# craftsangjae/instance-segmentation-road-project

Hardware: AMD Instinct MI355X
Metric: images/sec at 1024x1024 (MaskLab inference hot path, full forward) (higher is better)
Workload: dtype f32

## Files before the change

include/masklab_hip.h:

```cpp
#ifndef MASKLAB_HIP_H
#define MASKLAB_HIP_H

#include <stdint.h>

#ifdef __cplusplus
extern "C" {
#endif

#define ML_OK 0
#define ML_E_BADARG (-1)
#define ML_E_LAUNCH (-2)
#define ML_E_NOGPU  (-3)

enum { ML_ACT_NONE = 0, ML_ACT_RELU = 1, ML_ACT_RELU6 = 2, ML_ACT_SIGMOID = 3 };
enum { ML_MATH_F32 = 0, ML_MATH_F16 = 1, ML_MATH_F16S = 2, ML_MATH_F32X3 = 3 };

#define ML_ABI_VERSION 7
int ml_version(void);
const char *ml_last_error(void);
int ml_device_check(void);

typedef struct ml_conv2d_desc {
    const float *in;
    const float *wgt;
    const float *bias;
    const float *residual;
    float *out;
    int32_t B, H, W;
    int32_t in_cstride, in_coff;
    int32_t span;
    int32_t span_pad;
    int32_t cpp_shift;
    int32_t Ho, Wo;
    int32_t KH, KW, stride, dil, pad_t, pad_l;
    int32_t cout;
    int32_t n_pad;
    int32_t out_cstride, out_coff;
    int32_t res_cstride, res_coff;
    int32_t act;
    int32_t group_cin_step;
    int32_t shuffle2x2;
    int32_t tile;
    int32_t math;
    int32_t out_f16;
    int64_t out_bstride;
    const int32_t *live;
    int32_t live_period;
    int32_t reserved1;
    double *gn_partials;
} ml_conv2d_desc;

int ml_conv2d_f32(const ml_conv2d_desc *d, void *stream);

#define ML_CONV_MAX_PROBLEMS 12
int64_t ml_conv2d_workspace_bytes(void);
int ml_conv2d_multi_f32(const ml_conv2d_desc *descs, int32_t n, void *workspace, int64_t workspace_bytes,
                        void *stream);
int ml_conv2d_ntile(int32_t cout, int32_t tile);
int ml_conv2d_launch_ntile(const ml_conv2d_desc *descs, int32_t n, int32_t has_workspace);
int ml_conv2d_launch_mtile(const ml_conv2d_desc *descs, int32_t n, int32_t has_workspace);
int ml_conv2d_uses_pipe(const ml_conv2d_desc *d);
int ml_conv2d_launch_splits(const ml_conv2d_desc *descs, int32_t n, int64_t workspace_bytes, int32_t *splits);
int ml_conv2d_wino_eligible(const ml_conv2d_desc *d);
int64_t ml_conv2d_gn_min_launch_tiles(void);

int ml_gconv3x3_f32(const float *in, const float *wgt, const float *bias, float *out,
                    int32_t B, int32_t H, int32_t W, int32_t C, int32_t c, int32_t Ho, int32_t Wo,
                    int32_t stride, int32_t pad_t, int32_t pad_l, int32_t act, void *stream);

int ml_gconv3x3_f16(const void *in, const float *wgt, const float *bias, void *out,
                    int32_t B, int32_t H, int32_t W, int32_t C, int32_t c, int32_t Ho, int32_t Wo,
                    int32_t stride, int32_t pad_t, int32_t pad_l, int32_t act, void *stream);

int ml_maxpool3x3s2_f16(const void *in, void *out, int32_t B, int32_t H, int32_t W, int32_t C,
                        int32_t Ho, int32_t Wo, int32_t pad_t, int32_t pad_l, void *stream);
int ml_subsample2_f16(const void *in, void *out, int32_t B, int32_t H, int32_t W, int32_t C, void *stream);
int ml_cast_f16_to_f32(const void *in, float *out, int64_t n, void *stream);
int ml_cast_f32_to_f16(const float *in, void *out, int64_t n, void *stream);
int ml_resize_bilinear_ac_f16(const void *in, const void *add, void *out,
                              int32_t B, int32_t H, int32_t W, int32_t C, int32_t in_cstride, int32_t in_coff,
                              int32_t Ho, int32_t Wo, int32_t add_cstride, int32_t add_coff,
                              int32_t out_cstride, int32_t out_coff, void *stream);
int ml_dwconv3x3_f16(const void *in, const float *wgt, const float *bias, void *out,
                     int32_t B, int32_t H, int32_t W, int32_t C, int32_t in_cstride, int32_t in_coff,
                     int32_t out_cstride, int32_t out_coff, int32_t Ho, int32_t Wo,
                     int32_t stride, int32_t dil, int32_t pad_t, int32_t pad_l, int32_t act, void *stream);
int ml_global_mean_f16(const void *in, void *out, int32_t B, int32_t HW, int32_t C, void *stream);

int ml_stem7x7s2_pool_f16(const float *image, const void *wgt_h, const float *bias, void *out, int32_t B, int32_t H,
                          int32_t W, int32_t Hp, int32_t Wp, void *stream);
int ml_stem7x7s2_pool_f32(const float *image, const float *wgt, const float *bias, float *out, int32_t B, int32_t H,
                          int32_t W, int32_t Hp, int32_t Wp, void *stream);
int ml_stem7x7s2_pool_x3(const float *image, const void *wgt_x3, const float *bias, float *out, int32_t B, int32_t H,
                         int32_t W, int32_t Hp, int32_t Wp, void *stream);

typedef struct ml_deconv_out_problem {
    const float *x, *wd, *bd, *wo_table, *bo;
    float *out;
    int64_t M;
    int32_t hw, w, rois_per_image, reserved0;
    int64_t out_image_stride, out_base;
    const int32_t *live;
} ml_deconv_out_problem;
int ml_deconv2x2_out1x1_f32(const ml_deconv_out_problem *probs, int32_t nprob, int32_t K, int32_t c_mid, int32_t ncls,
                            int32_t cp, int32_t act_mid, int32_t act_out, void *stream);
int ml_deconv2x2_out1x1_f16(const ml_deconv_out_problem *probs, int32_t nprob, int32_t K, int32_t c_mid, int32_t ncls,
                            int32_t cp, int32_t act_mid, int32_t act_out, void *stream);

int ml_dwconv3x3_f32(const float *in, const float *wgt, const float *bias, float *out,
                     int32_t B, int32_t H, int32_t W, int32_t C,
                     int32_t in_cstride, int32_t in_coff, int32_t out_cstride, int32_t out_coff,
                     int32_t Ho, int32_t Wo, int32_t stride, int32_t dil,
                     int32_t pad_t, int32_t pad_l, int32_t act, void *stream);

int ml_maxpool3x3s2_f32(const float *in, float *out, int32_t B, int32_t H, int32_t W, int32_t C,
                        int32_t Ho, int32_t Wo, int32_t pad_t, int32_t pad_l, void *stream);
// ... 259 lines not shown
```

instance-segmentation-road-project_amd/csrc/conv_wino.hip:

```cpp
#include "common.h"

namespace {

constexpr int WMAXP = ML_CONV_MAX_PROBLEMS;
constexpr int WT = 64;
constexpr int WN = 64;
constexpr int WK = 8;
constexpr int WCHUNK = WK * 32 * 16;
constexpr int WSTEP = 4 * 32 * 16;
constexpr int NSLOT_P = 3;
constexpr int SLOT_P = WT * 16 * 8;
constexpr int NSLOT_W = 4;
constexpr int SLOT_W = 2 * WSTEP;
constexpr int RING_W = NSLOT_P * SLOT_P;
constexpr int LDS_BYTES = (RING_W + NSLOT_W * SLOT_W) * 4;
static_assert(LDS_BYTES == 160 * 1024, "the two rings fill the CU's LDS");
#ifndef WINO_EXP
#define WINO_EXP 0
#endif
constexpr unsigned OOB = 0x80000000u;
constexpr long long SPAN_MAX = 0x7fffff00ll;

struct WProblem {
    ml_conv2d_desc d;
    int TH, TW, T;
    int MB, NB, nchunks;
};

struct WArgs {
    int n;
    int start[WMAXP + 1];
    WProblem p[WMAXP];
};

__device__ __forceinline__ void dma16(__amdgpu_buffer_rsrc_t rsrc, float *dst, int voff) {
#if defined(__HIP_DEVICE_COMPILE__)
    __builtin_amdgcn_raw_ptr_buffer_load_lds(rsrc, (__attribute__((address_space(3))) void *)dst, 16, voff, 0, 0, 0);
#endif
}

__device__ __forceinline__ void bt_d_b_op(int k, const float d[16], float t[16], float v[16]) {
    if (k < 16) {
        const int j = k >> 2;
        switch (k & 3) {
            case 0: t[0 * 4 + j] = d[0 * 4 + j] - d[2 * 4 + j]; break;
            case 1: t[1 * 4 + j] = d[1 * 4 + j] + d[2 * 4 + j]; break;
            case 2: t[2 * 4 + j] = d[2 * 4 + j] - d[1 * 4 + j]; break;
            default: t[3 * 4 + j] = d[1 * 4 + j] - d[3 * 4 + j]; break;
        }
    } else {
        const int i = (k - 16) >> 2;
        switch (k & 3) {
            case 0: v[i * 4 + 0] = t[i * 4 + 0] - t[i * 4 + 2]; break;
            case 1: v[i * 4 + 1] = t[i * 4 + 1] + t[i * 4 + 2]; break;
            case 2: v[i * 4 + 2] = t[i * 4 + 2] - t[i * 4 + 1]; break;
            default: v[i * 4 + 3] = t[i * 4 + 1] - t[i * 4 + 3]; break;
        }
    }
}

__global__ void __launch_bounds__(512, 1) conv_wino_kernel(const WArgs args) {
    extern __shared__ __align__(16) float lds[];

    int pi = 0;
    while (pi + 1 < args.n && (int)blockIdx.x >= args.start[pi + 1]) ++pi;
    const WProblem &P = args.p[pi];
    const ml_conv2d_desc &p = P.d;
    const int b = (int)blockIdx.x - args.start[pi];
    const int g = b / (8 * P.NB), rr = b - g * 8 * P.NB;
    const int nt2 = rr >> 3;
    const int mt = g * 8 + (rr & 7);
    if (mt >= P.MB) return;
    if (p.live) {
        const int lv = max(1, *p.live), tpi0 = P.TH * P.TW;
        const int b0 = mt * WT / tpi0, b1 = min(mt * WT + WT, P.T) - 1;
        bool any = false;
        for (int bi = b0; bi <= b1 / tpi0 && !any; ++bi) any = bi % p.live_period < lv;
        if (!any) return;
    }

    const int tid = threadIdx.x, lane = tid & 63;
    const int wave = __builtin_amdgcn_readfirstlane(tid >> 6);
    const int tg = wave & 3, h = wave >> 2;
    const int r = lane & 15, kq = lane >> 4;
    const int tpi = P.TH * P.TW;

    const int gt0 = mt * WT;
    long long base_pix;
    {
        const int bi = gt0 / tpi, rem = gt0 - bi * tpi, ty = rem / P.TW;
        base_pix = ((long long)bi * p.H + max(2 * ty - 1, 0)) * p.W;
    }
    const size_t cstride = (size_t)p.in_cstride;
    const float *pin = p.in + p.in_coff + (size_t)base_pix * cstride;
    int voff_p[4];
    {
        const int rt = (lane >> 1) & 15;
        const int quad = (lane & 1) ^ ((rt >> 2) & 1);
        const int gt = gt0 + (wave >> 1) * 16 + rt;
        int bi = 0, ty = 0, tx = 0;
        if (gt < P.T) {
            bi = gt / tpi;
            const int rem = gt - bi * tpi;
            ty = rem / P.TW;
            tx = rem - ty * P.TW;
        }
#pragma unroll
        for (int i = 0; i < 4; ++i) {
            const int px = 8 * (wave & 1) + 2 * i + (lane >> 5);
            const int y = 2 * ty - 1 + (px >> 2), x = 2 * tx - 1 + (px & 3);
            voff_p[i] = (int)OOB;
            if (gt < P.T && y >= 0 && y < p.H && x >= 0 && x < p.W)
                voff_p[i] = (int)((((long long)bi * p.H + y) * p.W + x - base_pix) * (long long)cstride * 4) + quad * 16;
        }
    }
    const int voff_w = ((wave & 3) * 512 + r * 16 + kq * 4) * 4;
    const float *wsrc = p.wgt + (size_t)(2 * nt2 + (wave >> 2)) * P.nchunks * WCHUNK;
    float *dst_p = lds + (wave >> 1) * 2048 + (wave & 1) * 1024;
    float *dst_w = lds + RING_W + (wave >> 2) * WSTEP + (wave & 3) * 512;
    const int nch = P.nchunks, nsteps = 2 * P.nchunks;

    auto rsrc_p = [&](int j) __attribute__((always_inline)) {
        const bool real = j < nch && !(WINO_EXP & 1);
        return __builtin_amdgcn_make_buffer_rsrc((void *)(pin + j * 8), 0, real ? (int)OOB : 0, 0x00020000);
    };
    auto rsrc_w = [&](int s) __attribute__((always_inline)) {
        const bool real = s < nsteps && !(WINO_EXP & 2);
        return __builtin_amdgcn_make_buffer_rsrc((void *)(wsrc + (size_t)s * WSTEP), 0, real ? WSTEP * 4 : 0, 0x00020000);
    };

    f32x4 acc[2][16];
#pragma unroll
    for (int t = 0; t < 2; ++t)
#pragma unroll
        for (int q = 0; q < 16; ++q) acc[t][q] = f32x4{0.f, 0.f, 0.f, 0.f};

    const float *pa_lane0 = lds + tg * 2048 + r * 8 + 4 * ((r >> 2) & 1) + kq;
    const float *pa_lane1 = lds + tg * 2048 + r * 8 + 4 * (((r >> 2) & 1) ^ 1) + kq;
    const float *pb_lane = lds + RING_W + h * WSTEP + kq * 512 + r * 4;
    struct Ops {
        float d[16], t[16], v[16];
        f32x4 b[2][4];
    };
    auto read_ops = [&](const float *pa, const float *pb, Ops &o) __attribute__((always_inline)) {
#pragma unroll
        for (int t = 0; t < 2; ++t)
#pragma unroll
            for (int pq = 0; pq < 4; ++pq) o.b[t][pq] = *reinterpret_cast<const f32x4 *>(pb + t * 256 + pq * 64);
#pragma unroll
        for (int px = 0; px < 16; ++px) o.d[px] = pa[px * 128];
    };

    auto step = [&](const Ops &cur, Ops &nxt, const float *pa, const float *pb, const int ndma, auto dma) __attribute__((always_inline)) {
#if WINO_EXP == 4
#pragma unroll
        for (int q = 0; q < ndma; ++q) dma(q);
        __builtin_amdgcn_sched_barrier(0);
#endif
#pragma unroll
        for (int m = 0; m < 32; ++m) {
            const int t = m >> 4, pq = (m >> 2) & 3, e = m & 3;
            acc[t][4 * pq + e] =
                __builtin_amdgcn_mfma_f32_16x16x4f32(cur.v[4 * pq + e], cur.b[t][pq][e], acc[t][4 * pq + e], 0, 0, 0);
            if (m == 3) {
                __builtin_amdgcn_sched_barrier(0);
                read_ops(pa, pb, nxt);
                __builtin_amdgcn_sched_barrier(0);
            }
#if WINO_EXP != 4
            if (m % 6 == 5 && m / 6 < ndma) {
                __builtin_amdgcn_sched_barrier(0);
                dma(m / 6);
                __builtin_amdgcn_sched_barrier(0);
            }
#endif
            if (m >= 16) {
                bt_d_b_op(2 * (m - 16), nxt.d, nxt.t, nxt.v);
                bt_d_b_op(2 * (m - 16) + 1, nxt.d, nxt.t, nxt.v);
                __builtin_amdgcn_sched_barrier(0);
            }
        }
    };

    {
        const __amdgpu_buffer_rsrc_t rp0 = rsrc_p(0), rp1 = rsrc_p(1), rw0 = rsrc_w(0), rw1 = rsrc_w(1), rw2 = rsrc_w(2);
#pragma unroll
        for (int i = 0; i < 4; ++i) dma16(rp0, dst_p + i * 256, voff_p[i]);
        dma16(rw0, dst_w, voff_w);
        dma16(rw0, dst_w + 256, voff_w + 1024);
#pragma unroll
        for (int i = 0; i < 4; ++i) dma16(rp1, dst_p + SLOT_P + i * 256, voff_p[i]);
        dma16(rw1, dst_w + SLOT_W, voff_w);
        dma16(rw1, dst_w + SLOT_W + 256, voff_w + 1024);
        dma16(rw2, dst_w + 2 * SLOT_W, voff_w);
        dma16(rw2, dst_w + 2 * SLOT_W + 256, voff_w + 1024);
    }
    Ops oa, ob;
    asm volatile("s_waitcnt vmcnt(8)" ::: "memory");
    __builtin_amdgcn_s_barrier();
    read_ops(pa_lane0, pb_lane, oa);
#pragma unroll
    for (int k = 0; k < 32; ++k) bt_d_b_op(k, oa.d, oa.t, oa.v);

    int ps0 = 0, ps1 = SLOT_P, ps2 = 2 * SLOT_P;
    for (int j = 0; j < nch; ++j) {
        const int w0 = (2 * j) & 3;
        const int wa = ((w0 ^ 2) + 1) * SLOT_W, wb = w0 * SLOT_W;
        asm volatile("s_waitcnt vmcnt(0) lgkmcnt(0)" ::: "memory");
        __builtin_amdgcn_s_barrier();
        const __amdgpu_buffer_rsrc_t rp = rsrc_p(j + 2), rwa = rsrc_w(2 * j + 3), rwb = rsrc_w(2 * j + 4);
        auto dma = [&](int q) __attribute__((always_inline)) {
            if (q < 4) dma16(rp, dst_p + ps2 + q * 256, voff_p[q]);
            else if (q < 6) dma16(rwa, dst_w + wa + (q - 4) * 256, voff_w + (q - 4) * 1024);
            else dma16(rwb, dst_w + wb + (q - 6) * 256, voff_w + (q - 6) * 1024);
        };
        step(oa, ob, pa_lane1 + ps0, pb_lane + (w0 + 1) * SLOT_W, 5, dma);
        step(ob, oa, pa_lane0 + ps1, pb_lane + (w0 ^ 2) * SLOT_W, 3, [&](int q) __attribute__((always_inline)) { dma(q + 5); });
        const int ps = ps0;
        ps0 = ps1;
        ps1 = ps2;
        ps2 = ps;
    }
    asm volatile("s_waitcnt vmcnt(0)" ::: "memory");

    const int nt = 2 * nt2 + h;
    const bool gn = p.gn_partials != nullptr;
    double gs[2] = {0.0, 0.0}, gq[2] = {0.0, 0.0};
    long long f0 = 0;
    if (gn) {
        const int bi = gt0 / tpi, rem = gt0 - bi * tpi, ty = rem / P.TW, tx = rem - ty * P.TW;
        f0 = ((long long)(bi * p.Ho + 2 * ty) * p.Wo + 2 * tx) >> 7;
    }
    const float lo = 0.f, hi = (p.act == ML_ACT_RELU6) ? 6.f : 3.402823466e38f;
    const bool clampv = p.act == ML_ACT_RELU || p.act == ML_ACT_RELU6;
#pragma unroll
    for (int i = 0; i < 4; ++i) {
        const int gt = gt0 + tg * 16 + kq * 4 + i;
        if (gt >= P.T) continue;
        const int bi = gt / tpi, rem = gt - bi * tpi;
        const int ty = rem / P.TW, tx = rem - ty * P.TW;
        const int oy = 2 * ty, ox = 2 * tx;
        const bool y1 = oy + 1 < p.Ho, x1 = ox + 1 < p.Wo;
        const size_t img = p.out_bstride ? (size_t)bi * (size_t)p.out_bstride : (size_t)bi * p.Ho * p.Wo * p.out_cstride;
        const size_t pix0 = (size_t)oy * p.Wo + ox;
#pragma unroll
        for (int t = 0; t < 2; ++t) {
            const int n = nt * 32 + 16 * t + r;
            if (n >= p.cout) continue;
            float m[16];
#pragma unroll
            for (int q = 0; q < 16; ++q) m[q] = acc[t][q][i];
            float u[8];
#pragma unroll
            for (int j = 0; j < 4; ++j) {
                u[j] = m[0 * 4 + j] + m[1 * 4 + j] + m[2 * 4 + j];
                u[4 + j] = m[1 * 4 + j] - m[2 * 4 + j] - m[3 * 4 + j];
            }
            float yv[4];
#pragma unroll
            for (int a = 0; a < 2; ++a) {
                yv[2 * a] = u[4 * a + 0] + u[4 * a + 1] + u[4 * a + 2];
                yv[2 * a + 1] = u[4 * a + 1] - u[4 * a + 2] - u[4 * a + 3];
            }
            const float bv = p.bias ? p.bias[n] : 0.f;
            float *o = p.out + img + p.out_coff + n;
#pragma unroll
            for (int a = 0; a < 2; ++a)
#pragma unroll
                for (int c2 = 0; c2 < 2; ++c2) {
                    if ((a && !y1) || (c2 && !x1)) continue;
                    float val = yv[2 * a + c2] + bv;
                    if (clampv) val = __builtin_amdgcn_fmed3f(val, lo, hi);
                    else if (p.act != ML_ACT_NONE) val = ml_apply_act(val, p.act);
                    o[(pix0 + (size_t)a * p.Wo + c2) * p.out_cstride] = val;
                    if (gn) {
                        const long long m_flat = ((long long)(bi * p.Ho + oy + a) * p.Wo + ox + c2);
                        const int f = (m_flat >> 7) != f0;
                        gs[f] += (double)val;
                        gq[f] += (double)val * (double)val;
                    }
                }
        }
    }
    if (gn) {
        double *lds_gn = reinterpret_cast<double *>(lds);
        __syncthreads();
#pragma unroll
        for (int o = 32; o > 0; o >>= 1) {
#pragma unroll
            for (int f = 0; f < 2; ++f) {
                gs[f] += __shfl_down(gs[f], o, 64);
                gq[f] += __shfl_down(gq[f], o, 64);
            }
        }
        if (lane == 0) {
            lds_gn[wave * 4 + 0] = gs[0]; lds_gn[wave * 4 + 1] = gq[0];
            lds_gn[wave * 4 + 2] = gs[1]; lds_gn[wave * 4 + 3] = gq[1];
        }
        __syncthreads();
        if (tid < 4) {
            const int hh = tid >> 1, ff = tid & 1;
            const int gt1 = gt0 + WT - 1;
            const int bi = gt1 / tpi, rem = gt1 - bi * tpi, ty = rem / P.TW, tx = rem - ty * P.TW;
            const long long f1 = ((long long)(bi * p.Ho + 2 * ty + 1) * p.Wo + 2 * tx + 1) >> 7;
            const long long ft = ff ? f1 : f0;
            const int slot = 2 * nt2 + hh;
            double s = 0.0, q = 0.0;
            for (int w = 0; w < 4; ++w) { s += lds_gn[(hh * 4 + w) * 4 + 2 * ff]; q += lds_gn[(hh * 4 + w) * 4 + 2 * ff + 1]; }
            p.gn_partials[2 * (ft * 4 + slot)] = s;
            p.gn_partials[2 * (ft * 4 + slot) + 1] = q;
        }
    }
}

}

extern "C" int ml_conv2d_wino_eligible(const ml_conv2d_desc *d) {
    if (!d) return 0;
    return d->math == ML_MATH_F32 && d->KH == 3 && d->KW == 3 && d->stride == 1 && d->dil == 1 && d->pad_t == 1 &&
           d->pad_l == 1 && d->Ho == d->H && d->Wo == d->W && d->cpp_shift == 30 && d->group_cin_step == 0 &&
           !d->shuffle2x2 && !d->residual && !d->out_f16 && d->span % 32 == 0 && d->span_pad == d->span &&
           d->cout <= 128 && d->n_pad == 128;
}

int ml_conv2d_wino_gn_ok(const ml_conv2d_desc &d) {
    if (d.Ho % 2 || d.Wo % 2 || d.cout != 128 || d.out_bstride || d.act == ML_ACT_SIGMOID) return 0;
    const long long TH = d.Ho / 2, TW = d.Wo / 2;
    return (64 % TW == 0 || TW % 64 == 0) && (TH * TW) % 64 == 0;
}

int ml_conv2d_wino_launch(const ml_conv2d_desc *descs, int n, hipStream_t s) {
    ML_REQUIRE(n >= 1 && n <= WMAXP, "conv2d (winograd): need 1..%d problems", WMAXP);
    WArgs args;
    args.n = n;
    long long start = 0;
    for (int i = 0; i < n; ++i) {
        const ml_conv2d_desc &d = descs[i];
        ML_REQUIRE(ml_conv2d_wino_eligible(&d),
                   "conv2d: tile = 6 (Winograd F(2x2,3x3)) needs ML_MATH_F32, a 3x3 stride-1 undilated 'same' conv, no "
                   "groups / shuffle / residual / half output, span %% 32 == 0 and n_pad == 128");
        ML_REQUIRE(((d.in_cstride | d.in_coff) & 3) == 0 && ml_aligned16(d.in) && ml_aligned16(d.wgt),
                   "conv2d (winograd): 16-byte aligned input channels and weights");
        if (d.gn_partials)
            ML_REQUIRE(ml_conv2d_wino_gn_ok(d) && !d.live, "conv2d (winograd): gn_partials needs even Ho / Wo, Wo / 2 dividing or a "
                                                "multiple of 64, (Ho / 2) (Wo / 2) %% 64 == 0, cout = 128, dense output");
        WProblem &P = args.p[i];
        P.d = d;
        P.TH = (d.Ho + 1) / 2;
        P.TW = (d.Wo + 1) / 2;
        const long long T = (long long)d.B * P.TH * P.TW;
        ML_REQUIRE(T < (1ll << 30), "conv2d (winograd): too many tiles");
        P.T = (int)T;
        P.MB = (int)((T + WT - 1) / WT);
        P.NB = d.n_pad / WN;
        P.nchunks = d.span_pad / WK;
        const long long span = (2ll * (WT / P.TW + 2) + 2) * d.W * d.in_cstride * 4;
        ML_REQUIRE(span <= SPAN_MAX, "conv2d (winograd): a block's input rows exceed 2 GiB (W x in_cstride too large)");
        args.start[i] = (int)start;
        start += (long long)(P.MB + 7) / 8 * 8 * P.NB;
        ML_REQUIRE(start < (1ll << 31), "conv2d (winograd): grid too large");
    }
    args.start[n] = (int)start;
    long long tiles128 = 0;
    bool any_gn = false;
    for (int i = 0; i < n; ++i) {
        tiles128 += ((long long)descs[i].B * descs[i].Ho * descs[i].Wo + 127) / 128 * (descs[i].n_pad / 128);
        any_gn = any_gn || descs[i].gn_partials != nullptr;
    }
    ML_REQUIRE(!any_gn || tiles128 >= ml_conv2d_gn_min_launch_tiles(),
               "conv2d (winograd): gn_partials needs a launch of ml_conv2d_gn_min_launch_tiles() tiles of 128 x 128");
    static std::atomic<unsigned long long> lds_ok{0};
    if (int rc = ml_ensure_dynamic_lds(reinterpret_cast<const void *>(conv_wino_kernel), LDS_BYTES, lds_ok, "conv2d (winograd)"))
        return rc;
    hipLaunchKernelGGL(conv_wino_kernel, dim3((unsigned)start), dim3(512), LDS_BYTES, s, args);
    ML_CHECK_LAUNCH("conv2d (winograd)");
    return ML_OK;
}
```

instance-segmentation-road-project_amd/masklab_hip/_lib.py:

```python
import ctypes as C
import os

_HERE = os.path.dirname(os.path.abspath(__file__))
LIB_PATH = os.path.join(_HERE, "libmasklab_hip.so")

ABI_VERSION = 7
ACT_NONE, ACT_RELU, ACT_RELU6, ACT_SIGMOID = 0, 1, 2, 3
ACT_BY_NAME = {None: ACT_NONE, "linear": ACT_NONE, "relu": ACT_RELU, "relu6": ACT_RELU6,
               "sigmoid": ACT_SIGMOID}


class ConvDesc(C.Structure):
    _fields_ = [
        ("in_", C.c_void_p), ("wgt", C.c_void_p), ("bias", C.c_void_p),
        ("residual", C.c_void_p), ("out", C.c_void_p),
        ("B", C.c_int32), ("H", C.c_int32), ("W", C.c_int32),
        ("in_cstride", C.c_int32), ("in_coff", C.c_int32),
        ("span", C.c_int32), ("span_pad", C.c_int32), ("cpp_shift", C.c_int32),
        ("Ho", C.c_int32), ("Wo", C.c_int32),
        ("KH", C.c_int32), ("KW", C.c_int32), ("stride", C.c_int32), ("dil", C.c_int32),
        ("pad_t", C.c_int32), ("pad_l", C.c_int32),
        ("cout", C.c_int32), ("n_pad", C.c_int32),
        ("out_cstride", C.c_int32), ("out_coff", C.c_int32),
        ("res_cstride", C.c_int32), ("res_coff", C.c_int32),
# ... 7 lines not shown

class GnDesc(C.Structure):
    _fields_ = [("x", C.c_void_p), ("y", C.c_void_p), ("gamma", C.c_void_p), ("beta", C.c_void_p),
                ("HWC", C.c_int64), ("N", C.c_int32), ("C", C.c_int32), ("G", C.c_int32), ("relu", C.c_int32),
                ("out_cstride", C.c_int32), ("out_coff", C.c_int32), ("eps", C.c_float), ("dtype", C.c_int32),
                ("live", C.c_void_p), ("live_period", C.c_int32), ("reserved", C.c_int32),
                ("partials", C.c_void_p), ("n_partials", C.c_int32), ("reserved2", C.c_int32)]


class DeconvOutProblem(C.Structure):
    _fields_ = [("x", C.c_void_p), ("wd", C.c_void_p), ("bd", C.c_void_p), ("wo_table", C.c_void_p),
                ("bo", C.c_void_p), ("out", C.c_void_p), ("M", C.c_int64), ("hw", C.c_int32), ("w", C.c_int32),
                ("rois_per_image", C.c_int32), ("reserved0", C.c_int32), ("out_image_stride", C.c_int64),
                ("out_base", C.c_int64), ("live", C.c_void_p)]


class SeDesc(C.Structure):
    _fields_ = [("x", C.c_void_p), ("out", C.c_void_p), ("w1", C.c_void_p), ("w2", C.c_void_p),
                ("B", C.c_int32), ("HW", C.c_int32), ("C", C.c_int32), ("Hd", C.c_int32),
                ("live", C.c_void_p), ("live_period", C.c_int32), ("reserved", C.c_int32), ("ws_offset", C.c_int64)]


class SeResidualDesc(C.Structure):
    _fields_ = [("x", C.c_void_p), ("shortcut", C.c_void_p), ("w1", C.c_void_p), ("b1", C.c_void_p),
                ("w2", C.c_void_p), ("b2", C.c_void_p), ("scale", C.c_void_p), ("shift", C.c_void_p),
                ("out_act", C.c_void_p), ("out_y", C.c_void_p),
                ("B", C.c_int32), ("HW", C.c_int32), ("C", C.c_int32), ("Hd", C.c_int32),
                ("mode", C.c_int32), ("reserved", C.c_int32)]


class SeBottleneckDesc(C.Structure):
    _fields_ = [("c3", C.c_void_p), ("residual", C.c_void_p), ("w1", C.c_void_p), ("b1", C.c_void_p),
                ("w2", C.c_void_p), ("b2", C.c_void_p), ("out", C.c_void_p),
                ("B", C.c_int32), ("HW", C.c_int32), ("C", C.c_int32), ("Hd", C.c_int32)]


SE_RES_GATE, SE_RES_BN_RELU = 0, 1
GN_MAX_PROBLEMS = 8
SE_MAX_PROBLEMS = 8
DECONV_OUT_MAX_PROBLEMS = 4
_i32, _i64, _f32, _vp = C.c_int32, C.c_int64, C.c_float, C.c_void_p

SIGNATURES = {
    "ml_version": (C.c_int, []),
    "ml_last_error": (C.c_char_p, []),
    "ml_device_check": (C.c_int, []),
    "ml_conv2d_f32": (C.c_int, [C.POINTER(ConvDesc), _vp]),
    "ml_conv2d_ntile": (C.c_int, [_i32, _i32]),
    "ml_conv2d_uses_pipe": (C.c_int, [C.POINTER(ConvDesc)]),
    "ml_conv2d_launch_ntile": (C.c_int, [C.POINTER(ConvDesc), _i32, _i32]),
    "ml_conv2d_launch_mtile": (C.c_int, [C.POINTER(ConvDesc), _i32, _i32]),
    "ml_conv2d_launch_splits": (C.c_int, [C.POINTER(ConvDesc), _i32, _i64, C.POINTER(C.c_int32)]),
    "ml_conv2d_wino_eligible": (C.c_int, [C.POINTER(ConvDesc)]),
    "ml_conv2d_gn_min_launch_tiles": (_i64, []),
    "ml_conv2d_workspace_bytes": (_i64, []),
    "ml_conv2d_multi_f32": (C.c_int, [C.POINTER(ConvDesc), _i32, _vp, _i64, _vp]),
    "ml_deconv2x2_out1x1_f32": (C.c_int, [C.POINTER(DeconvOutProblem), _i32, _i32, _i32, _i32, _i32, _i32, _i32, _vp]),
    "ml_gconv3x3_f32": (C.c_int, [_vp, _vp, _vp, _vp] + [_i32] * 11 + [_vp]),
    "ml_gconv3x3_f16": (C.c_int, [_vp, _vp, _vp, _vp] + [_i32] * 11 + [_vp]),
    "ml_maxpool3x3s2_f16": (C.c_int, [_vp, _vp] + [_i32] * 8 + [_vp]),
    "ml_stem7x7s2_pool_f16": (C.c_int, [_vp, _vp, _vp, _vp] + [_i32] * 5 + [_vp]),
    "ml_stem7x7s2_pool_f32": (C.c_int, [_vp, _vp, _vp, _vp] + [_i32] * 5 + [_vp]),
    "ml_stem7x7s2_pool_x3": (C.c_int, [_vp, _vp, _vp, _vp] + [_i32] * 5 + [_vp]),
    "ml_subsample2_f16": (C.c_int, [_vp, _vp] + [_i32] * 4 + [_vp]),
    "ml_cast_f16_to_f32": (C.c_int, [_vp, _vp, _i64, _vp]),
    "ml_cast_f32_to_f16": (C.c_int, [_vp, _vp, _i64, _vp]),
    "ml_resize_bilinear_ac_f16": (C.c_int, [_vp, _vp, _vp] + [_i32] * 12 + [_vp]),
    "ml_dwconv3x3_f16": (C.c_int, [_vp, _vp, _vp, _vp] + [_i32] * 15 + [_vp]),
    "ml_global_mean_f16": (C.c_int, [_vp, _vp, _i32, _i32, _i32, _vp]),
    "ml_groupnorm_chunk_f16": (C.c_int, [_vp, _vp, _vp, _vp, _i32, _i64, _i32, _i32, _f32, _i32, _i32, _i32, _vp, _vp]),
    "ml_roi_crop_resize_f16": (C.c_int, [_vp, _vp, _i32, _i32, _vp, _vp, _vp, _vp] + [_i32] * 10 + [_f32, _f32, _i32, _i32, _vp, _vp]),
    "ml_deconv2x2_out1x1_f16": (C.c_int, [C.POINTER(DeconvOutProblem), _i32, _i32, _i32, _i32, _i32, _i32, _i32, _vp]),
    "ml_dwconv3x3_f32": (C.c_int, [_vp, _vp, _vp, _vp] + [_i32] * 15 + [_vp]),
    "ml_maxpool3x3s2_f32": (C.c_int, [_vp, _vp] + [_i32] * 8 + [_vp]),
    "ml_preprocess_f32": (C.c_int, [_vp, _i32, _vp, _i64, _i32, _i32, C.POINTER(C.c_float), C.POINTER(C.c_float),
                                    C.POINTER(C.c_float), _vp]),
    "ml_groupnorm_workspace_bytes": (_i64, [_i32, _i32]),
    "ml_groupnorm_multi_f32": (C.c_int, [C.POINTER(GnDesc), _i32, _vp, _i64, _vp]),
    "ml_groupnorm_chunk_f32": (C.c_int, [_vp, _vp, _vp, _vp, _i32, _i64, _i32, _i32, _f32, _i32, _i32, _i32, _vp, _vp]),
    "ml_resize_bilinear_ac_f32": (C.c_int, [_vp, _vp, _vp] + [_i32] * 12 + [_vp]),
    "ml_global_mean_f32": (C.c_int, [_vp, _vp, _i32, _i32, _i32, _vp]),
    "ml_scale_channels_f32": (C.c_int, [_vp, _vp, _i32, _i32, _i32, _vp]),
    "ml_squeeze_excite_workspace_bytes": (_i64, [_i32, _i32, _i32]),
    "ml_squeeze_excite_f32": (C.c_int, [C.POINTER(SeDesc), _i32, _vp, _i64, _vp]),
    "ml_squeeze_excite_f16": (C.c_int, [C.POINTER(SeDesc), _i32, _vp, _i64, _vp]),
    "ml_se_residual_workspace_bytes": (_i64, [_i32, _i32, _i32]),
    "ml_se_residual_f32": (C.c_int, [C.POINTER(SeResidualDesc), _vp, _i64, _vp]),
    "ml_se_bottleneck_workspace_bytes": (_i64, [_i32, _i32, _i32]),
    "ml_se_bottleneck_f32": (C.c_int, [C.POINTER(SeBottleneckDesc), _vp, _i64, _vp]),
    "ml_se_bottleneck_f16": (C.c_int, [C.POINTER(SeBottleneckDesc), _vp, _i64, _vp]),
    "ml_conv1x1_dual_f32": (C.c_int, [_vp] * 5 + [_i32] * 7 + [_vp]),
    "ml_conv1x1_dual_f16": (C.c_int, [_vp] * 5 + [_i32] * 7 + [_vp]),
    "ml_restore_boxes_f32": (C.c_int, [_vp, _vp, _vp, _i32, _i32, _vp]),
    "ml_detection_workspace_bytes": (_i64, [_i32, _i32, _i32, _i32]),
    "ml_detection_proposal_f32": (C.c_int, [_vp, _vp, _vp, _vp, _vp, _vp, _i32, _i32, _i32, _f32, _f32, _f32, _i32, _vp, _vp]),
    "ml_mask_distribute_i32": (C.c_int, [_vp, _i32, _i32, _vp, _vp, _vp, _vp, _i32, _i32, _i32, _f32, _vp]),
    "ml_roi_crop_resize_f32": (C.c_int, [_vp, _vp, _i32, _i32, _vp, _vp, _vp, _vp] + [_i32] * 10 + [_f32, _f32, _i32, _i32, _vp, _vp]),
    "ml_mold_levels_f32": (C.c_int, [_vp, _vp, _i32, _i32, _i32, _i64, C.POINTER(C.c_int32), _vp]),
    "ml_mold_levels_dev_f32": (C.c_int, [_vp, _vp, _i32, _i32, _i32, _i64, _vp, _vp]),
    "ml_add_f32": (C.c_int, [_vp, _vp, _i64, _vp]),
    "ml_add_f16": (C.c_int, [_vp, _vp, _i64, _vp]),
    "ml_fill_f32": (C.c_int, [_vp, _f32, _i64, _vp]),
    "ml_resize_image_ac": (C.c_int, [_vp, _i32, _vp, _vp, _f32] + [_i32] * 6 + [_vp]),
    "ml_trim_instances_f32": (C.c_int, [_vp] * 5 + [_i32] * 5 + [_vp]),
    "ml_upsample_boxes_i32": (C.c_int, [_vp, _vp, _i64, _f32, _f32, _vp]),
    "ml_threshold_i32": (C.c_int, [_vp, _vp, _f32, _i64, _vp]),
# ... 81 lines not shown
```

instance-segmentation-road-project_amd/masklab_hip/ops.py:

```python
import ctypes as C
import threading

import numpy as np
import torch

from . import _lib
from .packing import PackedConv, pack_winograd, resolve_padding

import weakref

_ws_cache = {}
_ws_retired = []
_graph_owners = weakref.WeakSet()


def graph_owner_registered(model):
    _graph_owners.add(model)


def graph_owner_released(model):
    _graph_owners.discard(model)
    if not len(_graph_owners):
        _ws_retired.clear()

PROFILE = None
LAUNCH_LOG = None


class _Prof:
    def __init__(self, kernel, flops, nbytes, shape=""):
        self.on = PROFILE is not None
        if self.on:
            self.rec = {"kernel": kernel, "flops": float(flops), "bytes": float(nbytes), "shape": shape,
                        "start": torch.cuda.Event(enable_timing=True), "end": torch.cuda.Event(enable_timing=True)}

    def __enter__(self):
        if self.on:
            self.rec["start"].record()
        return self

    def __exit__(self, *exc):
        if self.on:
            self.rec["end"].record()
            PROFILE.append(self.rec)
        return False


CONV_MATH = "f32"
_MATH_CODE = {"f32": 0, "f16": 1, "f16s": 1, "f32x3": 3}


def set_conv_math(mode):
    global CONV_MATH
    if mode not in _MATH_CODE:
        raise ValueError(f"conv math must be one of {sorted(_MATH_CODE)}, got {mode!r}")
    CONV_MATH = mode


def dtype_label():
    return {"f32": "f32", "f32x3": "f32 tensors, products as 3 x f16 MFMA on split operands (22-bit), f32 accumulate",
            "f16": "f16 MFMA operands, f32 accumulate, f32 tensors",
            "f16s": "f16 MFMA, f32 accumulate, f16 tensors in backbone body and heads (f32 predictions)"}[CONV_MATH]


def _stream():
    return C.c_void_p(torch.cuda.current_stream().cuda_stream)


def _ptr(t):
    return C.c_void_p(t.data_ptr()) if t is not None else C.c_void_p(0)


def half_storage():
    return CONV_MATH == "f16s"


def _require_dev(t, name):
    if not isinstance(t, torch.Tensor) or not t.is_cuda:
        raise RuntimeError(f"masklab_hip: `{name}` must be a CUDA/HIP torch tensor -- the product path "
                           f"runs only on the MI355X kernels (no CPU fallback)")
    if not t.is_contiguous():
        raise RuntimeError(f"masklab_hip: `{name}` must be contiguous NHWC")


def workspace(nbytes, device, tag="ws"):
    key = (str(device), tag, torch.cuda.current_stream().cuda_stream)
    buf = _ws_cache.get(key)
    if buf is None or buf.numel() < nbytes:
        if buf is not None:
            _ws_retired.append(buf)
        buf = torch.empty(int(nbytes), dtype=torch.uint8, device=device)
        _ws_cache[key] = buf
    return buf


class DeviceConv:

    def __init__(self, packed: PackedConv, device):
        self.p = packed
        self.wgt = torch.from_numpy(np.ascontiguousarray(packed.wgt)).to(device)
        self.bias = None if packed.bias is None else torch.from_numpy(packed.bias).to(device)
        self._wgt_h = None
        self._wgt_x3 = None
        self._wgt_wino = None
        self._wgt_stem_h = None

    @property
    def wgt_wino(self):
        if self._wgt_wino is None:
# ... 1616 lines not shown
```

Measured before the change: 422.1.

## Make Winograd conv kernel persistent and prefetch the next tile across tile boundaries

Turns the Winograd conv kernel into a persistent kernel whose grid is capped at the number of resident blocks. Each block walks tiles in grid-strided order and starts the DMA for the next tile's first input and weight chunks while it finishes the current tile. This removes pipeline drain and refill at tile boundaries and per-block launch overhead. The cost is more register pressure for the next tile's geometry, a new requirement that n_pad is 128 with at least two chunks, and a test hook that caps the block count.

```diff
diff --git a/include/masklab_hip.h b/include/masklab_hip.h
--- a/include/masklab_hip.h
+++ b/include/masklab_hip.h
@@ -62,6 +62,7 @@
 int ml_conv2d_uses_pipe(const ml_conv2d_desc *d);
 int ml_conv2d_launch_splits(const ml_conv2d_desc *descs, int32_t n, int64_t workspace_bytes, int32_t *splits);
 int ml_conv2d_wino_eligible(const ml_conv2d_desc *d);
+int ml_conv2d_wino_set_max_blocks(int n);
 int64_t ml_conv2d_gn_min_launch_tiles(void);
 
 int ml_gconv3x3_f32(const float *in, const float *wgt, const float *bias, float *out,
diff --git a/instance-segmentation-road-project_amd/csrc/conv_wino.hip b/instance-segmentation-road-project_amd/csrc/conv_wino.hip
--- a/instance-segmentation-road-project_amd/csrc/conv_wino.hip
+++ b/instance-segmentation-road-project_amd/csrc/conv_wino.hip
@@ -62,39 +62,52 @@
 __global__ void __launch_bounds__(512, 1) conv_wino_kernel(const WArgs args) {
     extern __shared__ __align__(16) float lds[];
 
-    int pi = 0;
-    while (pi + 1 < args.n && (int)blockIdx.x >= args.start[pi + 1]) ++pi;
-    const WProblem &P = args.p[pi];
-    const ml_conv2d_desc &p = P.d;
-    const int b = (int)blockIdx.x - args.start[pi];
-    const int g = b / (8 * P.NB), rr = b - g * 8 * P.NB;
-    const int nt2 = rr >> 3;
-    const int mt = g * 8 + (rr & 7);
-    if (mt >= P.MB) return;
-    if (p.live) {
-        const int lv = max(1, *p.live), tpi0 = P.TH * P.TW;
-        const int b0 = mt * WT / tpi0, b1 = min(mt * WT + WT, P.T) - 1;
-        bool any = false;
-        for (int bi = b0; bi <= b1 / tpi0 && !any; ++bi) any = bi % p.live_period < lv;
-        if (!any) return;
-    }
+    const int total = args.start[args.n], G = (int)gridDim.x;
+    int live_pi = -1, live_lv = 1;
+    auto find = [&](int id, int &pi, int &mt, int &nt2) __attribute__((always_inline)) {
+        for (; id < total; id += G) {
+            while (pi + 1 < args.n && id >= args.start[pi + 1]) ++pi;
+            const WProblem &P = args.p[pi];
+            const int b = id - args.start[pi];
+            nt2 = (b >> 3) & 1;
+            mt = (b >> 4) * 8 + (b & 7);
+            if (mt >= P.MB) continue;
+            if (P.d.live) {
+                if (live_pi != pi) {
+                    live_lv = max(1, *P.d.live);
+                    live_pi = pi;
+                }
+                const int tpi0 = P.TH * P.TW;
+                const int b0 = mt * WT / tpi0, b1 = min(mt * WT + WT, P.T) - 1;
+                bool any = false;
+                for (int bi = b0; bi <= b1 / tpi0 && !any; ++bi) any = bi % P.d.live_period < live_lv;
+                if (!any) continue;
+            }
+            break;
+        }
+        return id;
+    };
+    int pi = 0, mt = 0, nt2 = 0;
+    const int id0 = find((int)blockIdx.x, pi, mt, nt2);
+    if (id0 >= total) return;
 
     const int tid = threadIdx.x, lane = tid & 63;
     const int wave = __builtin_amdgcn_readfirstlane(tid >> 6);
     const int tg = wave & 3, h = wave >> 2;
     const int r = lane & 15, kq = lane >> 4;
-    const int tpi = P.TH * P.TW;
-
-    const int gt0 = mt * WT;
-    long long base_pix;
-    {
-        const int bi = gt0 / tpi, rem = gt0 - bi * tpi, ty = rem / P.TW;
-        base_pix = ((long long)bi * p.H + max(2 * ty - 1, 0)) * p.W;
-    }
-    const size_t cstride = (size_t)p.in_cstride;
-    const float *pin = p.in + p.in_coff + (size_t)base_pix * cstride;
-    int voff_p[4];
-    {
+
+    auto geom = [&](int gpi, int gmt, int gnt2, int (&voff)[4], const float *&gpin, const float *&gwsrc, int &gnch)
+                    __attribute__((always_inline)) {
+        const WProblem &P = args.p[gpi];
+        const ml_conv2d_desc &p = P.d;
+        const int tpi = P.TH * P.TW, gt0 = gmt * WT;
+        long long base_pix;
+        {
+            const int bi = gt0 / tpi, rem = gt0 - bi * tpi, ty = rem / P.TW;
+            base_pix = ((long long)bi * p.H + max(2 * ty - 1, 0)) * p.W;
+        }
+        const size_t cstride = (size_t)p.in_cstride;
+        gpin = p.in + p.in_coff + (size_t)base_pix * cstride;
         const int rt = (lane >> 1) & 15;
         const int quad = (lane & 1) ^ ((rt >> 2) & 1);
         const int gt = gt0 + (wave >> 1) * 16 + rt;
@@ -109,24 +122,26 @@
         for (int i = 0; i < 4; ++i) {
             const int px = 8 * (wave & 1) + 2 * i + (lane >> 5);
             const int y = 2 * ty - 1 + (px >> 2), x = 2 * tx - 1 + (px & 3);
-            voff_p[i] = (int)OOB;
+            voff[i] = (int)OOB;
             if (gt < P.T && y >= 0 && y < p.H && x >= 0 && x < p.W)
-                voff_p[i] = (int)((((long long)bi * p.H + y) * p.W + x - base_pix) * (long long)cstride * 4) + quad * 16;
-        }
-    }
+                voff[i] = (int)((((long long)bi * p.H + y) * p.W + x - base_pix) * (long long)cstride * 4) + quad * 16;
+        }
+        gwsrc = p.wgt + (size_t)(2 * gnt2 + (wave >> 2)) * P.nchunks * WCHUNK;
+        gnch = P.nchunks;
+    };
     const int voff_w = ((wave & 3) * 512 + r * 16 + kq * 4) * 4;
-    const float *wsrc = p.wgt + (size_t)(2 * nt2 + (wave >> 2)) * P.nchunks * WCHUNK;
     float *dst_p = lds + (wave >> 1) * 2048 + (wave & 1) * 1024;
     float *dst_w = lds + RING_W + (wave >> 2) * WSTEP + (wave & 3) * 512;
-    const int nch = P.nchunks, nsteps = 2 * P.nchunks;
-
-    auto rsrc_p = [&](int j) __attribute__((always_inline)) {
-        const bool real = j < nch && !(WINO_EXP & 1);
-        return __builtin_amdgcn_make_buffer_rsrc((void *)(pin + j * 8), 0, real ? (int)OOB : 0, 0x00020000);
-    };
-    auto rsrc_w = [&](int s) __attribute__((always_inline)) {
-        const bool real = s < nsteps && !(WINO_EXP & 2);
-        return __builtin_amdgcn_make_buffer_rsrc((void *)(wsrc + (size_t)s * WSTEP), 0, real ? WSTEP * 4 : 0, 0x00020000);
+
+    int voff_p[4], voff_n[4], nch, nch_n = 0;
+    const float *pin, *wsrc, *pin_n, *wsrc_n;
+    geom(pi, mt, nt2, voff_p, pin, wsrc, nch);
+
+    auto rsrc_p = [&](const float *src, bool real) __attribute__((always_inline)) {
+        return __builtin_amdgcn_make_buffer_rsrc((void *)src, 0, real && !(WINO_EXP & 1) ? (int)OOB : 0, 0x00020000);
+    };
+    auto rsrc_w = [&](const float *src, bool real) __attribute__((always_inline)) {
+        return __builtin_amdgcn_make_buffer_rsrc((void *)src, 0, real && !(WINO_EXP & 2) ? WSTEP * 4 : 0, 0x00020000);
     };
 
     f32x4 acc[2][16];
@@ -183,7 +198,8 @@
     };
 
     {
-        const __amdgpu_buffer_rsrc_t rp0 = rsrc_p(0), rp1 = rsrc_p(1), rw0 = rsrc_w(0), rw1 = rsrc_w(1), rw2 = rsrc_w(2);
+        const __amdgpu_buffer_rsrc_t rp0 = rsrc_p(pin, true), rp1 = rsrc_p(pin + 8, true);
+        const __amdgpu_buffer_rsrc_t rw0 = rsrc_w(wsrc, true), rw1 = rsrc_w(wsrc + WSTEP, true), rw2 = rsrc_w(wsrc + 2 * WSTEP, true);
 #pragma unroll
         for (int i = 0; i < 4; ++i) dma16(rp0, dst_p + i * 256, voff_p[i]);
         dma16(rw0, dst_w, voff_w);
@@ -195,6 +211,14 @@
         dma16(rw2, dst_w + 2 * SLOT_W, voff_w);
         dma16(rw2, dst_w + 2 * SLOT_W + 256, voff_w + 1024);
     }
+    int pi_n = pi, mt_n = 0, nt2_n = 0;
+    int id_n = find(id0 + G, pi_n, mt_n, nt2_n);
+    bool has_n = id_n < total;
+    pin_n = pin;
+    wsrc_n = wsrc;
+#pragma unroll
+    for (int i = 0; i < 4; ++i) voff_n[i] = (int)OOB;
+    if (has_n) geom(pi_n, mt_n, nt2_n, voff_n, pin_n, wsrc_n, nch_n);
     Ops oa, ob;
     asm volatile("s_waitcnt vmcnt(8)" ::: "memory");
     __builtin_amdgcn_s_barrier();
@@ -203,114 +227,147 @@
     for (int k = 0; k < 32; ++k) bt_d_b_op(k, oa.d, oa.t, oa.v);
 
     int ps0 = 0, ps1 = SLOT_P, ps2 = 2 * SLOT_P;
-    for (int j = 0; j < nch; ++j) {
-        const int w0 = (2 * j) & 3;
-        const int wa = ((w0 ^ 2) + 1) * SLOT_W, wb = w0 * SLOT_W;
-        asm volatile("s_waitcnt vmcnt(0) lgkmcnt(0)" ::: "memory");
-        __builtin_amdgcn_s_barrier();
-        const __amdgpu_buffer_rsrc_t rp = rsrc_p(j + 2), rwa = rsrc_w(2 * j + 3), rwb = rsrc_w(2 * j + 4);
-        auto dma = [&](int q) __attribute__((always_inline)) {
-            if (q < 4) dma16(rp, dst_p + ps2 + q * 256, voff_p[q]);
-            else if (q < 6) dma16(rwa, dst_w + wa + (q - 4) * 256, voff_w + (q - 4) * 1024);
-            else dma16(rwb, dst_w + wb + (q - 6) * 256, voff_w + (q - 6) * 1024);
-        };
-        step(oa, ob, pa_lane1 + ps0, pb_lane + (w0 + 1) * SLOT_W, 5, dma);
-        step(ob, oa, pa_lane0 + ps1, pb_lane + (w0 ^ 2) * SLOT_W, 3, [&](int q) __attribute__((always_inline)) { dma(q + 5); });
-        const int ps = ps0;
-        ps0 = ps1;
-        ps1 = ps2;
-        ps2 = ps;
+    int sb = 0;
+    for (;;) {
+        const int nsteps = 2 * nch;
+        for (int j = 0; j < nch; ++j) {
+            const int w0 = (2 * j + sb) & 3;
+            const int wa = ((w0 ^ 2) + 1) * SLOT_W, wb = w0 * SLOT_W;
+            const bool nx = j + 2 >= nch;
+            if (j + 2 == nch) {
+#pragma unroll
+                for (int i = 0; i < 4; ++i) voff_p[i] = voff_n[i];
+            }
+            asm volatile("s_waitcnt vmcnt(0) lgkmcnt(0)" ::: "memory");
+            __builtin_amdgcn_s_barrier();
+            const int s3 = 2 * j + 3, s4 = 2 * j + 4;
+            const __amdgpu_buffer_rsrc_t rp = rsrc_p(nx ? pin_n + (j + 2 - nch) * 8 : pin + (j + 2) * 8, !nx || has_n);
+            const __amdgpu_buffer_rsrc_t rwa =
+                rsrc_w(s3 >= nsteps ? wsrc_n + (size_t)(s3 - nsteps) * WSTEP : wsrc + (size_t)s3 * WSTEP, s3 < nsteps || has_n);
+            const __amdgpu_buffer_rsrc_t rwb =
+                rsrc_w(s4 >= nsteps ? wsrc_n + (size_t)(s4 - nsteps) * WSTEP : wsrc + (size_t)s4 * WSTEP, s4 < nsteps || has_n);
+            auto dma = [&](int q) __attribute__((always_inline)) {
+                if (q < 4) dma16(rp, dst_p + ps2 + q * 256, voff_p[q]);
+                else if (q < 6) dma16(rwa, dst_w + wa + (q - 4) * 256, voff_w + (q - 4) * 1024);
+                else dma16(rwb, dst_w + wb + (q - 6) * 256, voff_w + (q - 6) * 1024);
+            };
+            step(oa, ob, pa_lane1 + ps0, pb_lane + (w0 + 1) * SLOT_W, 5, dma);
+            step(ob, oa, pa_lane0 + ps1, pb_lane + (w0 ^ 2) * SLOT_W, 3, [&](int q) __attribute__((always_inline)) { dma(q + 5); });
+            const int ps = ps0;
+            ps0 = ps1;
+            ps1 = ps2;
+            ps2 = ps;
+        }
+
+        const WProblem &P = args.p[pi];
+        const ml_conv2d_desc &p = P.d;
+        const int tpi = P.TH * P.TW, gt0 = mt * WT;
+        const int nt = 2 * nt2 + h;
+        const bool gn = p.gn_partials != nullptr;
+        double gs[2] = {0.0, 0.0}, gq[2] = {0.0, 0.0};
+        long long f0 = 0;
+        if (gn) {
+            const int bi = gt0 / tpi, rem = gt0 - bi * tpi, ty = rem / P.TW, tx = rem - ty * P.TW;
+            f0 = ((long long)(bi * p.Ho + 2 * ty) * p.Wo + 2 * tx) >> 7;
+        }
+        const float lo = 0.f, hi = (p.act == ML_ACT_RELU6) ? 6.f : 3.402823466e38f;
+        const bool clampv = p.act == ML_ACT_RELU || p.act == ML_ACT_RELU6;
+#pragma unroll
+        for (int i = 0; i < 4; ++i) {
+            const int gt = gt0 + tg * 16 + kq * 4 + i;
+            if (gt >= P.T) continue;
+            const int bi = gt / tpi, rem = gt - bi * tpi;
+            const int ty = rem / P.TW, tx = rem - ty * P.TW;
+            const int oy = 2 * ty, ox = 2 * tx;
+            const bool y1 = oy + 1 < p.Ho, x1 = ox + 1 < p.Wo;
+            const size_t img = p.out_bstride ? (size_t)bi * (size_t)p.out_bstride : (size_t)bi * p.Ho * p.Wo * p.out_cstride;
+            const size_t pix0 = (size_t)oy * p.Wo + ox;
+#pragma unroll
+            for (int t = 0; t < 2; ++t) {
+                const int n = nt * 32 + 16 * t + r;
+                if (n >= p.cout) continue;
+                float m[16];
+#pragma unroll
+                for (int q = 0; q < 16; ++q) m[q] = acc[t][q][i];
+                float u[8];
+#pragma unroll
+                for (int j = 0; j < 4; ++j) {
+                    u[j] = m[0 * 4 + j] + m[1 * 4 + j] + m[2 * 4 + j];
+                    u[4 + j] = m[1 * 4 + j] - m[2 * 4 + j] - m[3 * 4 + j];
+                }
+                float yv[4];
+#pragma unroll
+                for (int a = 0; a < 2; ++a) {
+                    yv[2 * a] = u[4 * a + 0] + u[4 * a + 1] + u[4 * a + 2];
+                    yv[2 * a + 1] = u[4 * a + 1] - u[4 * a + 2] - u[4 * a + 3];
+                }
+                const float bv = p.bias ? p.bias[n] : 0.f;
+                float *o = p.out + img + p.out_coff + n;
+#pragma unroll
+                for (int a = 0; a < 2; ++a)
+#pragma unroll
+                    for (int c2 = 0; c2 < 2; ++c2) {
+                        if ((a && !y1) || (c2 && !x1)) continue;
+                        float val = yv[2 * a + c2] + bv;
+                        if (clampv) val = __builtin_amdgcn_fmed3f(val, lo, hi);
+                        else if (p.act != ML_ACT_NONE) val = ml_apply_act(val, p.act);
+                        o[(pix0 + (size_t)a * p.Wo + c2) * p.out_cstride] = val;
+                        if (gn) {
+                            const long long m_flat = ((long long)(bi * p.Ho + oy + a) * p.Wo + ox + c2);
+                            const int f = (m_flat >> 7) != f0;
+                            gs[f] += (double)val;
+                            gq[f] += (double)val * (double)val;
+                        }
+                    }
+            }
+        }
+        if (gn) {
+            double *lds_gn = reinterpret_cast<double *>(lds + ps2);
+            __syncthreads();
+#pragma unroll
+            for (int o = 32; o > 0; o >>= 1) {
+#pragma unroll
+                for (int f = 0; f < 2; ++f) {
+                    gs[f] += __shfl_down(gs[f], o, 64);
+                    gq[f] += __shfl_down(gq[f], o, 64);
+                }
+            }
+            if (lane == 0) {
+                lds_gn[wave * 4 + 0] = gs[0]; lds_gn[wave * 4 + 1] = gq[0];
+                lds_gn[wave * 4 + 2] = gs[1]; lds_gn[wave * 4 + 3] = gq[1];
+            }
+            __syncthreads();
+            if (tid < 4) {
+                const int hh = tid >> 1, ff = tid & 1;
+                const int gt1 = gt0 + WT - 1;
+                const int bi = gt1 / tpi, rem = gt1 - bi * tpi, ty = rem / P.TW, tx = rem - ty * P.TW;
+                const long long f1 = ((long long)(bi * p.Ho + 2 * ty + 1) * p.Wo + 2 * tx + 1) >> 7;
+                const long long ft = ff ? f1 : f0;
+                const int slot = 2 * nt2 + hh;
+                double s = 0.0, q = 0.0;
+                for (int w = 0; w < 4; ++w) { s += lds_gn[(hh * 4 + w) * 4 + 2 * ff]; q += lds_gn[(hh * 4 + w) * 4 + 2 * ff + 1]; }
+                p.gn_partials[2 * (ft * 4 + slot)] = s;
+                p.gn_partials[2 * (ft * 4 + slot) + 1] = q;
+            }
+        }
+        if (!has_n) break;
+
+        sb = (sb + nsteps) & 3;
+        pi = pi_n;
+        mt = mt_n;
+        nt2 = nt2_n;
+        pin = pin_n;
+        wsrc = wsrc_n;
+        nch = nch_n;
+        id_n = find(id_n + G, pi_n, mt_n, nt2_n);
+        has_n = id_n < total;
+        if (has_n) geom(pi_n, mt_n, nt2_n, voff_n, pin_n, wsrc_n, nch_n);
+#pragma unroll
+        for (int t = 0; t < 2; ++t)
+#pragma unroll
+            for (int q = 0; q < 16; ++q) acc[t][q] = f32x4{0.f, 0.f, 0.f, 0.f};
     }
     asm volatile("s_waitcnt vmcnt(0)" ::: "memory");
-
-    const int nt = 2 * nt2 + h;
-    const bool gn = p.gn_partials != nullptr;
-    double gs[2] = {0.0, 0.0}, gq[2] = {0.0, 0.0};
-    long long f0 = 0;
-    if (gn) {
-        const int bi = gt0 / tpi, rem = gt0 - bi * tpi, ty = rem / P.TW, tx = rem - ty * P.TW;
-        f0 = ((long long)(bi * p.Ho + 2 * ty) * p.Wo + 2 * tx) >> 7;
-    }
-    const float lo = 0.f, hi = (p.act == ML_ACT_RELU6) ? 6.f : 3.402823466e38f;
-    const bool clampv = p.act == ML_ACT_RELU || p.act == ML_ACT_RELU6;
-#pragma unroll
-    for (int i = 0; i < 4; ++i) {
-        const int gt = gt0 + tg * 16 + kq * 4 + i;
-        if (gt >= P.T) continue;
-        const int bi = gt / tpi, rem = gt - bi * tpi;
-        const int ty = rem / P.TW, tx = rem - ty * P.TW;
-        const int oy = 2 * ty, ox = 2 * tx;
-        const bool y1 = oy + 1 < p.Ho, x1 = ox + 1 < p.Wo;
-        const size_t img = p.out_bstride ? (size_t)bi * (size_t)p.out_bstride : (size_t)bi * p.Ho * p.Wo * p.out_cstride;
-        const size_t pix0 = (size_t)oy * p.Wo + ox;
-#pragma unroll
-        for (int t = 0; t < 2; ++t) {
-            const int n = nt * 32 + 16 * t + r;
-            if (n >= p.cout) continue;
-            float m[16];
-#pragma unroll
-            for (int q = 0; q < 16; ++q) m[q] = acc[t][q][i];
-            float u[8];
-#pragma unroll
-            for (int j = 0; j < 4; ++j) {
-                u[j] = m[0 * 4 + j] + m[1 * 4 + j] + m[2 * 4 + j];
-                u[4 + j] = m[1 * 4 + j] - m[2 * 4 + j] - m[3 * 4 + j];
-            }
-            float yv[4];
-#pragma unroll
-            for (int a = 0; a < 2; ++a) {
-                yv[2 * a] = u[4 * a + 0] + u[4 * a + 1] + u[4 * a + 2];
-                yv[2 * a + 1] = u[4 * a + 1] - u[4 * a + 2] - u[4 * a + 3];
-            }
-            const float bv = p.bias ? p.bias[n] : 0.f;
-            float *o = p.out + img + p.out_coff + n;
-#pragma unroll
-            for (int a = 0; a < 2; ++a)
-#pragma unroll
-                for (int c2 = 0; c2 < 2; ++c2) {
-                    if ((a && !y1) || (c2 && !x1)) continue;
-                    float val = yv[2 * a + c2] + bv;
-                    if (clampv) val = __builtin_amdgcn_fmed3f(val, lo, hi);
-                    else if (p.act != ML_ACT_NONE) val = ml_apply_act(val, p.act);
-                    o[(pix0 + (size_t)a * p.Wo + c2) * p.out_cstride] = val;
-                    if (gn) {
-                        const long long m_flat = ((long long)(bi * p.Ho + oy + a) * p.Wo + ox + c2);
-                        const int f = (m_flat >> 7) != f0;
-                        gs[f] += (double)val;
-                        gq[f] += (double)val * (double)val;
-                    }
-                }
-        }
-    }
-    if (gn) {
-        double *lds_gn = reinterpret_cast<double *>(lds);
-        __syncthreads();
-#pragma unroll
-        for (int o = 32; o > 0; o >>= 1) {
-#pragma unroll
-            for (int f = 0; f < 2; ++f) {
-                gs[f] += __shfl_down(gs[f], o, 64);
-                gq[f] += __shfl_down(gq[f], o, 64);
-            }
-        }
-        if (lane == 0) {
-            lds_gn[wave * 4 + 0] = gs[0]; lds_gn[wave * 4 + 1] = gq[0];
-            lds_gn[wave * 4 + 2] = gs[1]; lds_gn[wave * 4 + 3] = gq[1];
-        }
-        __syncthreads();
-        if (tid < 4) {
-            const int hh = tid >> 1, ff = tid & 1;
-            const int gt1 = gt0 + WT - 1;
-            const int bi = gt1 / tpi, rem = gt1 - bi * tpi, ty = rem / P.TW, tx = rem - ty * P.TW;
-            const long long f1 = ((long long)(bi * p.Ho + 2 * ty + 1) * p.Wo + 2 * tx + 1) >> 7;
-            const long long ft = ff ? f1 : f0;
-            const int slot = 2 * nt2 + hh;
-            double s = 0.0, q = 0.0;
-            for (int w = 0; w < 4; ++w) { s += lds_gn[(hh * 4 + w) * 4 + 2 * ff]; q += lds_gn[(hh * 4 + w) * 4 + 2 * ff + 1]; }
-            p.gn_partials[2 * (ft * 4 + slot)] = s;
-            p.gn_partials[2 * (ft * 4 + slot) + 1] = q;
-        }
-    }
 }
 
 }
@@ -327,6 +384,14 @@
     if (d.Ho % 2 || d.Wo % 2 || d.cout != 128 || d.out_bstride || d.act == ML_ACT_SIGMOID) return 0;
     const long long TH = d.Ho / 2, TW = d.Wo / 2;
     return (64 % TW == 0 || TW % 64 == 0) && (TH * TW) % 64 == 0;
+}
+
+static std::atomic<int> wino_max_blocks{0};
+
+extern "C" int ml_conv2d_wino_set_max_blocks(int n) {
+    const int cap = n <= 0 ? 0 : (n < 8 ? 8 : n / 8 * 8);
+    wino_max_blocks.store(cap, std::memory_order_relaxed);
+    return cap;
 }
 
 int ml_conv2d_wino_launch(const ml_conv2d_desc *descs, int n, hipStream_t s) {
@@ -353,6 +418,7 @@
         P.T = (int)T;
         P.MB = (int)((T + WT - 1) / WT);
         P.NB = d.n_pad / WN;
+        ML_REQUIRE(P.NB == 2 && d.span_pad >= 2 * WK, "conv2d (winograd): n_pad == 128 and at least two 8-channel chunks");
         P.nchunks = d.span_pad / WK;
         const long long span = (2ll * (WT / P.TW + 2) + 2) * d.W * d.in_cstride * 4;
         ML_REQUIRE(span <= SPAN_MAX, "conv2d (winograd): a block's input rows exceed 2 GiB (W x in_cstride too large)");
@@ -372,7 +438,10 @@
     static std::atomic<unsigned long long> lds_ok{0};
     if (int rc = ml_ensure_dynamic_lds(reinterpret_cast<const void *>(conv_wino_kernel), LDS_BYTES, lds_ok, "conv2d (winograd)"))
         return rc;
-    hipLaunchKernelGGL(conv_wino_kernel, dim3((unsigned)start), dim3(512), LDS_BYTES, s, args);
+    const int cap = wino_max_blocks.load(std::memory_order_relaxed);
+    const long long resident = cap ? cap : ml_resident_blocks(1) / 8 * 8;
+    const unsigned grid = (unsigned)(start < resident ? start : resident);
+    hipLaunchKernelGGL(conv_wino_kernel, dim3(grid), dim3(512), LDS_BYTES, s, args);
     ML_CHECK_LAUNCH("conv2d (winograd)");
     return ML_OK;
 }
diff --git a/instance-segmentation-road-project_amd/masklab_hip/_lib.py b/instance-segmentation-road-project_amd/masklab_hip/_lib.py
--- a/instance-segmentation-road-project_amd/masklab_hip/_lib.py
+++ b/instance-segmentation-road-project_amd/masklab_hip/_lib.py
@@ -83,6 +83,7 @@
     "ml_conv2d_launch_mtile": (C.c_int, [C.POINTER(ConvDesc), _i32, _i32]),
     "ml_conv2d_launch_splits": (C.c_int, [C.POINTER(ConvDesc), _i32, _i64, C.POINTER(C.c_int32)]),
     "ml_conv2d_wino_eligible": (C.c_int, [C.POINTER(ConvDesc)]),
+    "ml_conv2d_wino_set_max_blocks": (C.c_int, [C.c_int]),
     "ml_conv2d_gn_min_launch_tiles": (_i64, []),
     "ml_conv2d_workspace_bytes": (_i64, []),
     "ml_conv2d_multi_f32": (C.c_int, [C.POINTER(ConvDesc), _i32, _vp, _i64, _vp]),
diff --git a/instance-segmentation-road-project_amd/masklab_hip/ops.py b/instance-segmentation-road-project_amd/masklab_hip/ops.py
--- a/instance-segmentation-road-project_amd/masklab_hip/ops.py
+++ b/instance-segmentation-road-project_amd/masklab_hip/ops.py
@@ -1,3 +1,4 @@
+import contextlib
 import ctypes as C
 import threading
 
@@ -55,6 +56,16 @@
     if mode not in _MATH_CODE:
         raise ValueError(f"conv math must be one of {sorted(_MATH_CODE)}, got {mode!r}")
     CONV_MATH = mode
+
+
+@contextlib.contextmanager
+def wino_max_blocks(n):
+    lib = _lib.load()
+    cap = lib.ml_conv2d_wino_set_max_blocks(int(n))
+    try:
+        yield cap
+    finally:
+        lib.ml_conv2d_wino_set_max_blocks(0)
 
 
 def dtype_label():
```

Measured after the change: 422.0. No clear change (-0.0%).
